# linhthi/BLISS-GNN

Measured on AMD Instinct MI355X. Metric: steps/sec (train step: sample_blocks + gather + SAGE fwd/bwd + Adam + exp3), reddit-like, higher is better.
Workload: dtype bf16

## Files before the change

bliss_gnn_amd/csrc/exp3.hip:

```cpp
#include "common.cuh"
#include "bliss_gnn.h"
#include "prof.h"
#include <cstdlib>

namespace {

#define E3_TPB 256
#ifndef NORM_NT
#define NORM_NT 1
#endif
#ifndef NORM_UNROLL
#define NORM_UNROLL 4
#endif

__device__ __forceinline__ void row_digits(bf16_t b, int64_t d[3], int* bad) {
  uint32_t e = (b >> 7) & 0xff, m = b & 0x7f;
  d[0] = d[1] = d[2] = 0;
  if (e == 255 || (b & 0x8000 && (b & 0x7fff))) { *bad |= BLISS_ERR_NONFINITE; return; }
  if (e == 0) e = 1; else m |= 0x80;
  int shift = (int)e - 134 + 64;
  if (shift > 80) { *bad |= BLISS_ERR_FIXED_RANGE; return; }
  if (shift < 0) { d[0] = (-shift >= 8) ? 0 : (int64_t)(m >> (-shift)); return; }
  const int idx = shift >> 5, off = shift & 31;
  const uint64_t v = (uint64_t)m << off;
  const int64_t lo = (int64_t)(v & 0xffffffffu), hi = (int64_t)(v >> 32);
  if (idx == 0) { d[0] = lo; d[1] = hi; }
  else if (idx == 1) { d[1] = lo; d[2] = hi; }
  else { d[2] = (int64_t)v; }
}

__device__ __forceinline__ int64_t wave_sum_i64(int64_t v) { return wave_total_i64(v); }

#define ROWSUM_SLOTS BLISS_ROWSUM_SLOTS
__device__ __forceinline__ void flush_digits(int64_t d[3], int64_t* limbs) {
  const int slot = (int)((blockIdx.x * (blockDim.x >> 6) + (threadIdx.x >> 6)) % ROWSUM_SLOTS);
#pragma unroll
  for (int i = 0; i < 3; ++i) {
    int64_t s = wave_sum_i64(d[i]);
    if (lane_id() == 0 && s != 0) atomicAdd((unsigned long long*)(limbs + 3 * slot + i), (unsigned long long)s);
  }
}
__device__ __forceinline__ void gather_limbs(const int64_t* limbs, int64_t out[3]) {
  out[0] = out[1] = out[2] = 0;
  for (int s = 0; s < ROWSUM_SLOTS; ++s) { out[0] += limbs[3 * s]; out[1] += limbs[3 * s + 1]; out[2] += limbs[3 * s + 2]; }
}

__device__ bf16_t limbs_to_bf16(const int64_t* replicas, int* bad) {
  int64_t limbs[3];
  gather_limbs(replicas, limbs);
  __int128 t = (__int128)limbs[0] + ((__int128)limbs[1] << 32) + ((__int128)limbs[2] << 64);
  if (t < 0) { *bad |= BLISS_ERR_FIXED_RANGE; return 0; }
  if (t == 0) return 0;
  unsigned __int128 u = (unsigned __int128)t;
  uint64_t hi = (uint64_t)(u >> 64), lo = (uint64_t)u;
  int msb = hi ? 127 - __clzll((long long)hi) : 63 - __clzll((long long)lo);
  unsigned __int128 q;
  if (msb > 7) {
    int sh = msb - 7;
    q = u >> sh;
    unsigned __int128 rem = u & ((((unsigned __int128)1) << sh) - 1), half = ((unsigned __int128)1) << (sh - 1);
    if (rem > half || (rem == half && (q & 1))) q += 1;
  } else q = u << (7 - msb);
  int e = msb - 64 + 127;
  if (q >= 256) { q >>= 1; e += 1; }
  if (e <= 0 || e >= 255) { *bad |= BLISS_ERR_FIXED_RANGE; return 0; }
  return (bf16_t)(((uint32_t)e << 7) | ((uint32_t)q & 0x7f));
}

__device__ __forceinline__ float nan_to_num_posinf0(float x) {
  if (x != x) return 0.f;
  if (x == __builtin_inff()) return 0.f;
  if (x == -__builtin_inff()) return -3.3895313892515355e38f;
  return x;
}

__device__ __forceinline__ void exp3_update_body(const int64_t* __restrict__ g_indptr, const bf16_t* __restrict__ edge_w,
                                                 bf16_t* w_row, int64_t* row_sum, const int* __restrict__ blk_indptr,
                                                 const int* __restrict__ blk_src, const int* __restrict__ blk_dst,
                                                 const int* __restrict__ blk_pos, const bf16_t* __restrict__ q_ij,
                                                 const bf16_t* __restrict__ node_prob, const bf16_t* __restrict__ embed_norm,
                                                 const bf16_t* __restrict__ alpha_in, const int* __restrict__ dst_nid,
                                                 const int* __restrict__ n_edges_dev, float delta_f,
                                                 bf16_t* __restrict__ rewards_out, bf16_t* __restrict__ factor_out,
                                                 int apply, int* err, int wg, int nwg, int bound) {
  int B = *n_edges_dev;
  int bad = 0;
  if (B > bound) { B = bound; bad |= BLISS_ERR_CAP_EDGES; }
  int64_t dg[3] = {0, 0, 0};
  for (int base = wg * E3_TPB + (threadIdx.x & ~63); base < B; base += nwg * E3_TPB) {
    const int e = base + lane_id();
    if (e < B) {
      const int i = blk_dst[e], j = blk_src[e], pos = blk_pos[e];
      const float alpha = bf2f(alpha_in ? alpha_in[e] : edge_w[pos]);
      const float k_i = rbf((float)(blk_indptr[i + 1] - blk_indptr[i]));
      float adk = rbf(rbf(alpha * alpha) / k_i);
      adk = nan_to_num_posinf0(adk);
      const float hn = bf2f(embed_norm[j]), q = bf2f(q_ij[e]);
      const float hq = rbf(rbf(hn * hn) / rbf(q * q));
      const float r = rbf(adk * hq);
      if (rewards_out) rewards_out[e] = f2bf(r);
      const int dn = dst_nid[i];
      const float n_i = rbf((float)(g_indptr[dn + 1] - g_indptr[dn]));
      const float r_hat = rbf(r / bf2f(node_prob[j]));
      float dr = rbf(r_hat * rbf(rbf(1.0f / n_i) * delta_f));
      if (dr > 1.0f) dr = 1.0f;
      const float ex = rbf((float)exp((double)dr));
      if (factor_out) factor_out[e] = f2bf(ex);
      if (!apply) continue;
      const bf16_t w_old = w_row[pos];
      const bf16_t w_new = f2bf(bf2f(w_old) * ex);
      if (w_new != w_old) {
        w_row[pos] = w_new;
        int64_t a[3], b[3];
        row_digits(w_new, a, &bad);
        row_digits(w_old, b, &bad);
        dg[0] += a[0] - b[0]; dg[1] += a[1] - b[1]; dg[2] += a[2] - b[2];
      }
    }
  }
  flush_digits(dg, row_sum);
  if (bad) atomicOr(err, bad);
}

__global__ void __launch_bounds__(E3_TPB) k_exp3_update(const int64_t* __restrict__ g_indptr, const bf16_t* __restrict__ edge_w,
                                                       bf16_t* w_row, int64_t* row_sum, const int* __restrict__ blk_indptr,
                                                       const int* __restrict__ blk_src, const int* __restrict__ blk_dst,
                                                       const int* __restrict__ blk_pos, const bf16_t* __restrict__ q_ij,
                                                       const bf16_t* __restrict__ node_prob, const bf16_t* __restrict__ embed_norm,
                                                       const bf16_t* __restrict__ alpha_in, const int* __restrict__ dst_nid,
                                                       const int* __restrict__ n_edges_dev, float delta_f,
                                                       bf16_t* __restrict__ rewards_out, bf16_t* __restrict__ factor_out,
                                                       int apply, int* err, int edges_bound) {
  exp3_update_body(g_indptr, edge_w, w_row, row_sum, blk_indptr, blk_src, blk_dst, blk_pos, q_ij, node_prob, embed_norm, alpha_in,
                   dst_nid, n_edges_dev, delta_f, rewards_out, factor_out, apply, err, blockIdx.x, gridDim.x, edges_bound);
}

struct Exp3Multi {
  bliss_exp3_block_t blk[BLISS_EXP3_MAX_BLOCKS];
  int grid_begin[BLISS_EXP3_MAX_BLOCKS + 1];
  int n;
};
__global__ void __launch_bounds__(E3_TPB) k_exp3_update_multi(const int64_t* __restrict__ g_indptr, const bf16_t* __restrict__ edge_w,
                                                             const Exp3Multi m, float delta_f, int* err) {
  int b = 0;
  while (b + 1 < m.n && (int)blockIdx.x >= m.grid_begin[b + 1]) ++b;
  const bliss_exp3_block_t& k = m.blk[b];
  exp3_update_body(g_indptr, edge_w, (bf16_t*)k.w_pos, k.row_sum, k.blk_indptr, k.blk_src, k.blk_dst, k.blk_pos, (const bf16_t*)k.q_ij,
                   (const bf16_t*)k.node_prob, (const bf16_t*)k.embed_norm, (const bf16_t*)k.alpha_or_null, k.dst_nid, k.n_edges_dev,
                   delta_f, (bf16_t*)k.rewards_out, nullptr, 1, err, (int)blockIdx.x - m.grid_begin[b], m.grid_begin[b + 1] - m.grid_begin[b],
                   k.edges_bound);
}

__global__ void __launch_bounds__(E3_TPB) k_exp3_apply(bf16_t* w_row, int64_t* row_sum, const int* __restrict__ pos,
                                                      const bf16_t* __restrict__ factor, const int* __restrict__ n_dev, int* err) {
  const int n = *n_dev;
  int bad = 0;
  int64_t dg[3] = {0, 0, 0};
  for (int e = blockIdx.x * E3_TPB + threadIdx.x; e < n; e += gridDim.x * E3_TPB) {
    const int p = pos[e];
    const bf16_t w_old = w_row[p];
    const bf16_t w_new = f2bf(bf2f(w_old) * bf2f(factor[e]));
    if (w_new != w_old) {
      w_row[p] = w_new;
      int64_t a[3], b[3];
      row_digits(w_new, a, &bad);
      row_digits(w_old, b, &bad);
      dg[0] += a[0] - b[0]; dg[1] += a[1] - b[1]; dg[2] += a[2] - b[2];
    }
  }
  flush_digits(dg, row_sum);
  if (bad) atomicOr(err, bad);
}

#define APPLY_MAX_WGS 256
struct ApplyLists {
  bf16_t* w_row[BLISS_EXP3_MAX_BLOCKS];
  int64_t* row_sum[BLISS_EXP3_MAX_BLOCKS];
  int pos_off[BLISS_EXP3_MAX_BLOCKS], fac_off[BLISS_EXP3_MAX_BLOCKS], cnt_off[BLISS_EXP3_MAX_BLOCKS], bound[BLISS_EXP3_MAX_BLOCKS];
  int n_blocks, n_ranks;
  long long rank_stride;
};

__global__ void __launch_bounds__(E3_TPB) k_exp3_apply_ranks(ApplyLists m, const int* __restrict__ gathered, int* bar, int* err) {
  int bad = 0;
  int64_t dg[BLISS_EXP3_MAX_BLOCKS][3];
#pragma unroll
  for (int b = 0; b < BLISS_EXP3_MAX_BLOCKS; ++b) dg[b][0] = dg[b][1] = dg[b][2] = 0;
  const int G = gridDim.x;
  for (int r = 0; r < m.n_ranks; ++r) {
    const int* base = gathered + (long long)r * m.rank_stride;
#pragma unroll
    for (int b = 0; b < BLISS_EXP3_MAX_BLOCKS; ++b) {
      if (b >= m.n_blocks) break;
      int n = base[m.cnt_off[b]];
      if (n > m.bound[b]) { n = m.bound[b]; bad |= BLISS_ERR_CAP_EDGES; }
      const int* pos = base + m.pos_off[b];
      const bf16_t* fac = reinterpret_cast<const bf16_t*>(base) + m.fac_off[b];
      for (int e = blockIdx.x * E3_TPB + threadIdx.x; e < n; e += G * E3_TPB) {
        const float f = bf2f(fac[e]);
        const uintptr_t a = (uintptr_t)(m.w_row[b] + pos[e]);
        unsigned* word = reinterpret_cast<unsigned*>(a & ~(uintptr_t)3);
        const int sh = (a & 2) ? 16 : 0;
        unsigned cur = __hip_atomic_load(word, __ATOMIC_RELAXED, __HIP_MEMORY_SCOPE_AGENT);
        for (;;) {
          const bf16_t w_old = (bf16_t)((cur >> sh) & 0xffffu);
          const bf16_t w_new = f2bf(bf2f(w_old) * f);
          if (w_new == w_old) break;
          const unsigned want = (cur & ~(0xffffu << sh)) | ((unsigned)w_new << sh);
          if (__hip_atomic_compare_exchange_strong(word, &cur, want, __ATOMIC_RELAXED, __ATOMIC_RELAXED, __HIP_MEMORY_SCOPE_AGENT)) {
            int64_t x[3], y[3];
            row_digits(w_new, x, &bad);
            row_digits(w_old, y, &bad);
            dg[b][0] += x[0] - y[0]; dg[b][1] += x[1] - y[1]; dg[b][2] += x[2] - y[2];
            break;
          }
        }
      }
    }
    if (r + 1 < m.n_ranks) {
      __syncthreads();
      if (threadIdx.x == 0) {
        __hip_atomic_fetch_add(bar, 1, __ATOMIC_RELEASE, __HIP_MEMORY_SCOPE_AGENT);
        long long spins = 0;
        while (__hip_atomic_load(bar, __ATOMIC_ACQUIRE, __HIP_MEMORY_SCOPE_AGENT) < (r + 1) * G) {
          __builtin_amdgcn_s_sleep(2);
          if (++spins > (1ll << 24)) { bad |= BLISS_ERR_FLAG_TIMEOUT; break; }
        }
      }
      __syncthreads();
    }
  }
#pragma unroll
  for (int b = 0; b < BLISS_EXP3_MAX_BLOCKS; ++b)
    if (b < m.n_blocks) flush_digits(dg[b], m.row_sum[b]);
  if (bad) atomicOr(err, bad);
  __syncthreads();
  if (threadIdx.x == 0 && __hip_atomic_fetch_add(bar + 1, 1, __ATOMIC_RELAXED, __HIP_MEMORY_SCOPE_AGENT) == G - 1) {
    __hip_atomic_store(bar, 0, __ATOMIC_RELAXED, __HIP_MEMORY_SCOPE_AGENT);
    __hip_atomic_store(bar + 1, 0, __ATOMIC_RELAXED, __HIP_MEMORY_SCOPE_AGENT);
  }
}

struct PackLists {
  const int* pos[BLISS_EXP3_MAX_BLOCKS];
  const int* n_dev[BLISS_EXP3_MAX_BLOCKS];
  int pos_off[BLISS_EXP3_MAX_BLOCKS], cnt_off[BLISS_EXP3_MAX_BLOCKS], bound[BLISS_EXP3_MAX_BLOCKS];
  int n_blocks;
};
__global__ void __launch_bounds__(E3_TPB) k_pack_lists(PackLists m, int* __restrict__ buf) {
  for (int b = 0; b < m.n_blocks; ++b) {
    const int n_true = *m.n_dev[b];
    const int n = n_true < m.bound[b] ? n_true : m.bound[b];
    if (blockIdx.x == 0 && threadIdx.x == 0) buf[m.cnt_off[b]] = n_true;
    const int* __restrict__ src = m.pos[b];
    int* __restrict__ dst = buf + m.pos_off[b];
    for (int e = blockIdx.x * E3_TPB + threadIdx.x; e < n; e += gridDim.x * E3_TPB) dst[e] = src[e];
  }
}

__global__ void __launch_bounds__(E3_TPB) k_row_sum(const bf16_t* __restrict__ w, int64_t n, int64_t* limbs, int* err) {
  int bad = 0;
  int64_t dg[3] = {0, 0, 0};
  for (int64_t i = (int64_t)blockIdx.x * E3_TPB + threadIdx.x; i < n; i += (int64_t)gridDim.x * E3_TPB) {
    int64_t a[3];
    row_digits(w[i], a, &bad);
    dg[0] += a[0]; dg[1] += a[1]; dg[2] += a[2];
  }
  flush_digits(dg, limbs);
  if (bad && err) atomicOr(err, bad);
}

__global__ void k_zero_i64(int64_t* p, int n) { if ((int)threadIdx.x < n) p[threadIdx.x] = 0; }

__device__ __forceinline__ float renorm_denom(bf16_t norm) { return rbf(fmaxf(bf2f(norm), 1e-12f)); }
__device__ __forceinline__ bf16_t renorm_bf16(bf16_t x, float denom) { return f2bf(bf2f(x) / denom); }

struct PairSlow { uint32_t word; int bad; int64_t d0, d1, d2; };
__device__ __attribute__((noinline)) PairSlow renorm_pair_slow(uint32_t word, float denom) {
  PairSlow r;
  r.bad = 0;
  const bf16_t lo = renorm_bf16((bf16_t)(word & 0xffffu), denom), hi = renorm_bf16((bf16_t)(word >> 16), denom);
  int64_t a[3], b[3];
  row_digits(lo, a, &r.bad);
  row_digits(hi, b, &r.bad);
  r.d0 = a[0] + b[0]; r.d1 = a[1] + b[1]; r.d2 = a[2] + b[2];
  r.word = (uint32_t)lo | ((uint32_t)hi << 16);
  return r;
}

__device__ __forceinline__ void normalize_row_body(bf16_t* w, int64_t n, int64_t* row_sum, int64_t* scratch, bf16_t* norm_out, int wg, int nwg,
                                                   const int64_t* norm_src = nullptr) {
  __shared__ int sh_norm, sh_last;
  if (threadIdx.x == 0) {
    int bad = 0;
    const bf16_t nb = limbs_to_bf16(norm_src ? norm_src : row_sum, &bad);
    sh_norm = (int)nb | (bad << 20);
    if (wg == 0) {
      scratch[0] = (int64_t)nb | ((int64_t)(nb == 0x3f80) << 16) | ((int64_t)bad << 20);
      if (norm_out) *norm_out = nb;
    }
  }
  __syncthreads();
  const bf16_t nb = (bf16_t)(sh_norm & 0xffff);
  if (nb == 0x3f80) return;
  const float denom = renorm_denom(nb);
  int bad = 0;
  int64_t dg[3] = {0, 0, 0};
  __shared__ int sh_tbl[128];
  if (threadIdx.x < 128) {
    const bf16_t x0 = (bf16_t)(0x3f80u | threadIdx.x);
    sh_tbl[threadIdx.x] = ((int)renorm_bf16(x0, denom) - (int)x0) & 0xffff;
  }
  const int de_lo = (int)(renorm_bf16((bf16_t)0x3f80u, denom) >> 7) - 127;
  const int de_hi = (int)(renorm_bf16((bf16_t)0x3fffu, denom) >> 7) - 127;
  const bool tbl_ok = de_lo > -126 && de_hi < 126 && de_lo <= de_hi;
  const uint32_t e_lo = (uint32_t)max(2, 2 - de_lo), e_hi = (uint32_t)min(253, 253 - de_hi);
  const int f_lo = max((int)e_lo, 70 - de_lo), f_hi = min((int)e_hi, 125 - de_hi);
  const bool pair_ok = tbl_ok && e_hi >= e_lo && f_hi >= f_lo;
  typedef unsigned short u16x2 __attribute__((ext_vector_type(2)));
  const unsigned short f_base = pair_ok ? (unsigned short)f_lo : (unsigned short)0xffffu, f_span = pair_ok ? (unsigned short)(f_hi - f_lo) : (unsigned short)0;
  const u16x2 FLO2 = {f_base, f_base}, SPAN2 = {f_span, f_span};
  __shared__ unsigned sh_bins[7][E3_TPB];
#pragma unroll
  for (int a = 0; a < 7; ++a) sh_bins[a][threadIdx.x] = 0;
  __syncthreads();
  auto one = [&](bf16_t x) {
    const bf16_t v = renorm_bf16(x, denom);
    int64_t a[3];
    row_digits(v, a, &bad);
    dg[0] += a[0]; dg[1] += a[1]; dg[2] += a[2];
    return v;
  };
  const int64_t head = min(n, (int64_t)(((16 - ((uintptr_t)w & 15)) & 15) >> 1));
  const int64_t nvec = (n - head) / 8;
  const int64_t gtid = (int64_t)wg * E3_TPB + threadIdx.x, gsz = (int64_t)nwg * E3_TPB;
  if (gtid < head) w[gtid] = one(w[gtid]);
  for (int64_t i = head + nvec * 8 + gtid; i < n; i += gsz) w[i] = one(w[i]);
  typedef unsigned int u32x4 __attribute__((ext_vector_type(4)));
  u32x4* wv = reinterpret_cast<u32x4*>(w + head);
#pragma unroll NORM_UNROLL
  for (int64_t i = gtid; i < nvec; i += gsz) {
#if NORM_NT
    u32x4 x = __builtin_nontemporal_load(wv + i);
#else
    u32x4 x = wv[i];
#endif
#pragma unroll
    for (int k = 0; k < 4; ++k) {
      const uint32_t word = x[k];
      const u16x2 W = __builtin_bit_cast(u16x2, word);
      const u16x2 D = (W >> 7) - FLO2;
      if (__builtin_bit_cast(uint32_t, __builtin_elementwise_max(D, SPAN2)) == __builtin_bit_cast(uint32_t, SPAN2)) {
        const uint32_t t = (uint32_t)sh_tbl[word & 0x7fu] | ((uint32_t)sh_tbl[(word >> 16) & 0x7fu] << 16);
        const u16x2 V = W + __builtin_bit_cast(u16x2, t);
        const uint32_t v2 = __builtin_bit_cast(uint32_t, V);
        const u16x2 S = (V >> 7) - (u16x2){70, 70};
        const u16x2 M = __builtin_bit_cast(u16x2, (v2 & 0x007f007fu) | 0x00800080u);
        const u16x2 T = M << (S & (u16x2){7, 7});
        const u16x2 A = S >> 3;
        __hip_atomic_fetch_add(&sh_bins[A.x][threadIdx.x], (unsigned)T.x, __ATOMIC_RELAXED, __HIP_MEMORY_SCOPE_WORKGROUP);
        __hip_atomic_fetch_add(&sh_bins[A.y][threadIdx.x], (unsigned)T.y, __ATOMIC_RELAXED, __HIP_MEMORY_SCOPE_WORKGROUP);
        x[k] = v2;
      } else {
        const PairSlow r = renorm_pair_slow(word, denom);
        x[k] = r.word; bad |= r.bad;
        dg[0] += r.d0; dg[1] += r.d1; dg[2] += r.d2;
      }
    }
#if NORM_NT == 1
    __builtin_nontemporal_store(x, wv + i);
#else
    wv[i] = x;
#endif
  }
  {
    uint64_t a = 0, b = 0;
#pragma unroll
    for (int k = 0; k < 4; ++k) a += (uint64_t)sh_bins[k][threadIdx.x] << (8 * k);
#pragma unroll
    for (int k = 4; k < 7; ++k) b += (uint64_t)sh_bins[k][threadIdx.x] << (8 * (k - 4));
    dg[0] += (int64_t)(a & 0xffffffffull); dg[1] += (int64_t)(a >> 32);
    dg[1] += (int64_t)(b & 0xffffffffull); dg[2] += (int64_t)(b >> 32);
  }
  flush_digits(dg, scratch + 2);
  if (bad) atomicOr((unsigned long long*)scratch, (unsigned long long)bad << 20);
  asm volatile("s_waitcnt vmcnt(0)" ::: "memory");
  __syncthreads();
  if (threadIdx.x == 0) sh_last = (atomicAdd((unsigned long long*)(scratch + 1), 1ull) == (unsigned long long)nwg - 1);
  __syncthreads();
  if (sh_last) {
    for (int k = threadIdx.x; k < 3 * ROWSUM_SLOTS; k += E3_TPB) {
      row_sum[k] = (int64_t)__hip_atomic_load((unsigned long long*)(scratch + 2 + k), __ATOMIC_RELAXED, __HIP_MEMORY_SCOPE_AGENT);
      __hip_atomic_store((unsigned long long*)(scratch + 2 + k), 0ull, __ATOMIC_RELAXED, __HIP_MEMORY_SCOPE_AGENT);
    }
    if (threadIdx.x == 0) __hip_atomic_store((unsigned long long*)(scratch + 1), 0ull, __ATOMIC_RELAXED, __HIP_MEMORY_SCOPE_AGENT);
  }
}

__global__ void __launch_bounds__(E3_TPB) k_normalize_row(bf16_t* w, int64_t n, int64_t* row_sum, int64_t* scratch, bf16_t* norm_out,
                                                          const int64_t* norm_src) {
  normalize_row_body(w, n, row_sum, scratch, norm_out, blockIdx.x, gridDim.x, norm_src);
}
__global__ void __launch_bounds__(E3_TPB) k_normalize_rows_global(const Exp3Multi m, int64_t n, int per_row, const int64_t* __restrict__ limbs,
                                                                  int64_t limb_stride) {
  const int r = blockIdx.x / per_row;
  const bliss_exp3_block_t& k = m.blk[r];
  normalize_row_body((bf16_t*)k.w_pos, n, k.row_sum, k.scratch, (bf16_t*)k.norm_out, (int)blockIdx.x - r * per_row, per_row, limbs + r * limb_stride);
}
__global__ void __launch_bounds__(E3_TPB) k_normalize_rows(const Exp3Multi m, int64_t n, int per_row) {
  const int r = blockIdx.x / per_row;
  const bliss_exp3_block_t& k = m.blk[r];
  normalize_row_body((bf16_t*)k.w_pos, n, k.row_sum, k.scratch, (bf16_t*)k.norm_out, (int)blockIdx.x - r * per_row, per_row);
}

__global__ void __launch_bounds__(E3_TPB) k_normalized_edata(const int64_t* __restrict__ indptr, int num_nodes, bf16_t* __restrict__ out) {
  const int lane = lane_id();
  for (int v = blockIdx.x * (E3_TPB / 64) + (threadIdx.x >> 6); v < num_nodes; v += gridDim.x * (E3_TPB / 64)) {
    const int64_t b = indptr[v], e = indptr[v + 1];
    const bf16_t val = f2bf(1.0f / rbf((float)(e - b)));
    for (int64_t p = b + lane; p < e; p += 64) out[p] = val;
  }
}

}

static int norm_wgs() {
  static const int v = [] { const char* e = getenv("BLISS_NORM_WGS"); int x = e ? atoi(e) : 0; return x > 0 ? x : 1024; }();
  return v;
}

extern "C" {

int bliss_exp3_update(const bliss_graph_t* g, const void* edge_w_pos, void* w_pos, int64_t* row_sum,
                      const int32_t* blk_indptr, const int32_t* blk_src, const int32_t* blk_dst,
                      const int32_t* blk_pos, const void* q_ij, const void* node_prob, const void* embed_norm,
                      const void* alpha_or_null, const int32_t* dst_nid, int32_t n_dst, const int32_t* n_edges_dev,
                      int32_t edges_bound, float delta_f, void* rewards_out, void* factor_out, int apply,
                      int32_t* err, void* stream) {
  if (!g || !w_pos || !row_sum || !blk_indptr || !blk_src || !blk_dst || !blk_pos || !q_ij || !node_prob ||
      !embed_norm || !dst_nid || !n_edges_dev || !err || (!edge_w_pos && !alpha_or_null))
    return BLISS_EINVAL;
  (void)n_dst;
  if (edges_bound <= 0) return 0;
  int grid = (edges_bound + E3_TPB - 1) / E3_TPB;
  if (grid > 2048) grid = 2048;
  hipStream_t st = (hipStream_t)stream;
  PROF_LAUNCH(BK_EXP3_UPDATE, st, k_exp3_update<<<grid, E3_TPB, 0, st>>>(g->indptr, (const bf16_t*)edge_w_pos, (bf16_t*)w_pos, row_sum, blk_indptr,
                                                          blk_src, blk_dst, blk_pos, (const bf16_t*)q_ij, (const bf16_t*)node_prob,
                                                          (const bf16_t*)embed_norm, (const bf16_t*)alpha_or_null, dst_nid,
                                                          n_edges_dev, delta_f, (bf16_t*)rewards_out, (bf16_t*)factor_out, apply, err, edges_bound));
  return (int)hipGetLastError();
}
// ... 160 lines not shown
```

bliss_gnn_amd/csrc/spmm.hip:

```cpp
#include "common.cuh"
#include "bliss_gnn.h"
#include "prof.h"

extern "C" int bliss_spmm_chunk_edges(int32_t nnz_bound);

namespace {

#define SP_TPB 256

struct f4 { float x, y, z, w; };

__device__ __forceinline__ int bcast_i(int v, int j) { return __builtin_amdgcn_readlane(v, j); }
__device__ __forceinline__ float bcast_f(float v, int j) { return __int_as_float(__builtin_amdgcn_readlane(__float_as_int(v), j)); }

__device__ __forceinline__ f4 load4(const bf16_t* p) {
  uint2 v = *reinterpret_cast<const uint2*>(p);
  f4 r;
  r.x = __uint_as_float(v.x << 16); r.y = __uint_as_float(v.x & 0xffff0000u);
  r.z = __uint_as_float(v.y << 16); r.w = __uint_as_float(v.y & 0xffff0000u);
  return r;
}

template <bool OUT_F32>
__device__ __forceinline__ void store4(void* out, int64_t off, f4 a) {
  if (OUT_F32) {
    *reinterpret_cast<float4*>((float*)out + off) = make_float4(a.x, a.y, a.z, a.w);
  } else {
    uint2 v;
    v.x = (uint32_t)f2bf(a.x) | ((uint32_t)f2bf(a.y) << 16);
    v.y = (uint32_t)f2bf(a.z) | ((uint32_t)f2bf(a.w) << 16);
    *reinterpret_cast<uint2*>((bf16_t*)out + off) = v;
  }
}


template <bool VEC4, bool OUT_F32>
__device__ __forceinline__ void store_row(void* out, int64_t off, f4 a, float scale) {
  a.x *= scale; a.y *= scale; a.z *= scale; a.w *= scale;
  if (VEC4) store4<OUT_F32>(out, off, a);
  else if (OUT_F32) ((float*)out)[off] = a.x;
  else ((bf16_t*)out)[off] = f2bf(a.x);
}

template <bool VEC4, bool OUT_F32, bool BWD>
__global__ void __launch_bounds__(SP_TPB) k_spmm(const int* __restrict__ row_ptr, const int* __restrict__ t_edge,
                                                const int* __restrict__ src, const int* __restrict__ dst,
                                                const int* __restrict__ blk_indptr, const bf16_t* __restrict__ w,
                                                const bf16_t* __restrict__ h, int64_t h_stride, int n_rows,
                                                const int* __restrict__ nnz_dev, int nnz_host, int dim,
                                                int mean, void* out, int64_t out_stride, float* __restrict__ part, int EC) {
  const int nnz = nnz_dev ? min(*nnz_dev, nnz_host) : nnz_host;
  const int lane = lane_id();
  const int chunk = blockIdx.x * (SP_TPB / 64) + (threadIdx.x >> 6);
  const int nchunks = nnz > 0 ? (nnz + EC - 1) / EC : 1;
  if (chunk >= nchunks) return;
  const int c0 = chunk * EC, c1 = min(nnz, c0 + EC), cnt = c1 - c0;
  int my_row = -1, my_n = 0;
  float my_c = 0.f;
  if (lane < cnt) {
    const int e = BWD ? t_edge[c0 + lane] : c0 + lane;
    my_row = BWD ? src[e] : dst[e];
    my_n = BWD ? dst[e] : src[e];
    float c = w ? bf2f(w[e]) : 1.0f;
    if (BWD && mean) { const int d = dst[e]; c = c / (float)max(blk_indptr[d + 1] - blk_indptr[d], 1); }
    my_c = c;
  }
  constexpr int W = VEC4 ? 4 : 1;
  const f4 zero = {0.f, 0.f, 0.f, 0.f};
  for (int col0 = 0; col0 < dim; col0 += 64 * W) {
    const int col = col0 + lane * W;
    const bool act = col < dim;
    auto flush = [&](int r, f4 acc) {
      const int rb = row_ptr[r], re = row_ptr[r + 1];
      const bool starts = rb >= c0, ends = re <= c1;
      if (!act) return;
      if (starts && ends) {
        const float scale = (!BWD && mean) ? 1.0f / (float)max(re - rb, 1) : 1.0f;
        store_row<VEC4, OUT_F32>(out, r * out_stride + col, acc, scale);
      } else {
        float* q = part + ((int64_t)chunk * 2 + (starts ? 1 : 0)) * dim + col;
        q[0] = acc.x;
        if (VEC4) { q[1] = acc.y; q[2] = acc.z; q[3] = acc.w; }
      }
    };
    if (cnt == 0) continue;
    int cur = bcast_i(my_row, 0);
    f4 acc = zero;
    for (int j = 0; j < cnt;) {
      const int r = bcast_i(my_row, j);
      if (r != cur) { flush(cur, acc); acc = zero; cur = r; }
      const int run = __popcll(__ballot(my_row == r && lane >= j));
      const int end = j + run;
      for (; j + 4 <= end; j += 4) {
        int n0 = bcast_i(my_n, j), n1 = bcast_i(my_n, j + 1), n2 = bcast_i(my_n, j + 2), n3 = bcast_i(my_n, j + 3);
        float k0 = bcast_f(my_c, j), k1 = bcast_f(my_c, j + 1), k2 = bcast_f(my_c, j + 2), k3 = bcast_f(my_c, j + 3);
        if (act) {
          if (VEC4) {
            f4 a0 = load4(h + n0 * h_stride + col), a1 = load4(h + n1 * h_stride + col);
            f4 a2 = load4(h + n2 * h_stride + col), a3 = load4(h + n3 * h_stride + col);
            acc.x += k0 * a0.x; acc.y += k0 * a0.y; acc.z += k0 * a0.z; acc.w += k0 * a0.w;
            acc.x += k1 * a1.x; acc.y += k1 * a1.y; acc.z += k1 * a1.z; acc.w += k1 * a1.w;
            acc.x += k2 * a2.x; acc.y += k2 * a2.y; acc.z += k2 * a2.z; acc.w += k2 * a2.w;
            acc.x += k3 * a3.x; acc.y += k3 * a3.y; acc.z += k3 * a3.z; acc.w += k3 * a3.w;
          } else {
            float a0 = bf2f(h[n0 * h_stride + col]), a1 = bf2f(h[n1 * h_stride + col]);
            float a2 = bf2f(h[n2 * h_stride + col]), a3 = bf2f(h[n3 * h_stride + col]);
            acc.x += k0 * a0; acc.x += k1 * a1; acc.x += k2 * a2; acc.x += k3 * a3;
          }
        }
      }
      for (; j < end; ++j) {
        int n0 = bcast_i(my_n, j);
        float k0 = bcast_f(my_c, j);
        if (act) {
          if (VEC4) {
            f4 a0 = load4(h + n0 * h_stride + col);
            acc.x += k0 * a0.x; acc.y += k0 * a0.y; acc.z += k0 * a0.z; acc.w += k0 * a0.w;
          } else acc.x += k0 * bf2f(h[n0 * h_stride + col]);
        }
      }
    }
    flush(cur, acc);
  }
}

template <bool OUT_F32, bool BWD, bool VEC4>
__global__ void __launch_bounds__(SP_TPB) k_spmm_fixup(const int* __restrict__ row_ptr, int n_rows, int dim, int mean,
                                                      const float* __restrict__ part, void* out, int64_t out_stride, int EC) {
  const int lane = lane_id();
  const int r = blockIdx.x * (SP_TPB / 64) + (threadIdx.x >> 6);
  if (r >= n_rows) return;
  const int rb = row_ptr[r], re = row_ptr[r + 1];
  constexpr int W = VEC4 ? 4 : 1;
  const f4 zero = {0.f, 0.f, 0.f, 0.f};
  if (re <= rb) {
    for (int col = lane * W; col < dim; col += 64 * W) store_row<VEC4, OUT_F32>(out, r * out_stride + col, zero, 1.0f);
    return;
  }
  const int c = rb / EC, c_end = (re - 1) / EC;
  if (c_end == c) return;
  const float scale = (!BWD && mean) ? 1.0f / (float)(re - rb) : 1.0f;
  for (int col = lane * W; col < dim; col += 64 * W) {
    f4 sum = zero;
    if (VEC4) {
      const float4 v = *reinterpret_cast<const float4*>(part + ((int64_t)c * 2 + 1) * dim + col);
      sum.x = v.x; sum.y = v.y; sum.z = v.z; sum.w = v.w;
#pragma unroll 4
      for (int cc = c + 1; cc <= c_end; ++cc) {
        const float4 u = *reinterpret_cast<const float4*>(part + ((int64_t)cc * 2) * dim + col);
        sum.x += u.x; sum.y += u.y; sum.z += u.z; sum.w += u.w;
      }
    } else {
      sum.x = part[((int64_t)c * 2 + 1) * dim + col];
      for (int cc = c + 1; cc <= c_end; ++cc) sum.x += part[((int64_t)cc * 2) * dim + col];
    }
    store_row<VEC4, OUT_F32>(out, r * out_stride + col, sum, scale);
  }
}

__global__ void __launch_bounds__(SP_TPB) k_embed_norm(const bf16_t* __restrict__ h, int n_rows, int dim, int64_t stride,
                                                      bf16_t* __restrict__ out, int vec4) {
  const int lane = lane_id();
  const int row = blockIdx.x * (SP_TPB / 64) + (threadIdx.x >> 6);
  if (row >= n_rows) return;
  const bf16_t* p = h + row * stride;
  float s = 0.f;
  if (vec4) {
    for (int c = lane * 4; c < dim; c += 256) {
      f4 a = load4(p + c);
      s += a.x * a.x; s += a.y * a.y; s += a.z * a.z; s += a.w * a.w;
    }
  } else {
    for (int c = lane; c < dim; c += 64) { float a = bf2f(p[c]); s += a * a; }
  }
  for (int d = 32; d >= 1; d >>= 1) s += __shfl_xor(s, d);
  if (lane == 0) out[row] = f2bf(sqrtf(s));
}

template <int W>
__global__ void __launch_bounds__(SP_TPB) k_gather_rows_norm(const bf16_t* __restrict__ feat, int64_t f_stride, const int* __restrict__ ids,
                                                            int n_rows, int dim, bf16_t* __restrict__ out, int64_t o_stride,
                                                            bf16_t* __restrict__ norm_out, int norm_vec4) {
  extern __shared__ __attribute__((aligned(16))) bf16_t rows_sh[];
  const int lane = lane_id(), wave = threadIdx.x >> 6;
  const int row = blockIdx.x * (SP_TPB / 64) + wave;
  if (row >= n_rows) return;
  const int dpad = (dim + 7) & ~7;
  bf16_t* sh = rows_sh + (size_t)wave * dpad;
  const bf16_t* p = feat + (int64_t)ids[row] * f_stride;
  bf16_t* q = out + (int64_t)row * o_stride;
  if (W == 4) {
    for (int c = lane * 4; c < dim; c += 256) { const uint2 v = *reinterpret_cast<const uint2*>(p + c); *reinterpret_cast<uint2*>(q + c) = v; *reinterpret_cast<uint2*>(sh + c) = v; }
  } else if (W == 2) {
    for (int c = lane * 2; c < dim; c += 128) { const uint32_t v = *reinterpret_cast<const uint32_t*>(p + c); *reinterpret_cast<uint32_t*>(q + c) = v; *reinterpret_cast<uint32_t*>(sh + c) = v; }
  } else {
    for (int c = lane; c < dim; c += 64) { const bf16_t v = p[c]; q[c] = v; sh[c] = v; }
  }
  if (!norm_out) return;
  __builtin_amdgcn_fence(__ATOMIC_RELEASE, "wavefront");
  __builtin_amdgcn_wave_barrier();
  float s = 0.f;
  if (norm_vec4) {
    for (int c = lane * 4; c < dim; c += 256) {
      const float a = bf2f(sh[c]), b = bf2f(sh[c + 1]), cc = bf2f(sh[c + 2]), d = bf2f(sh[c + 3]);
      s += a * a; s += b * b; s += cc * cc; s += d * d;
    }
  } else {
    for (int c = lane; c < dim; c += 64) { const float a = bf2f(sh[c]); s += a * a; }
  }
  for (int d = 32; d >= 1; d >>= 1) s += __shfl_xor(s, d);
  if (lane == 0) norm_out[row] = f2bf(sqrtf(s));
}

__device__ __forceinline__ uint32_t drop_hash(uint32_t seed, uint32_t ctr, uint32_t idx) {
  uint32_t x = idx * 0x9e3779b1u + seed;
  x ^= ctr * 0x85ebca77u + 0x165667b1u;
  x ^= x >> 16; x *= 0x7feb352du; x ^= x >> 15; x *= 0x846ca68bu; x ^= x >> 16;
  x += ctr; x ^= x >> 15; x *= 0x2c1b3c6du; x ^= x >> 12;
  return x;
}

template <bool VEC4>
__global__ void __launch_bounds__(SP_TPB) k_sage_epilogue(const bf16_t* __restrict__ a, int64_t a_stride, const bf16_t* __restrict__ b,
                                                         int64_t b_stride, int n_rows, int dim, uint32_t drop_thresh, float scale,
                                                         uint32_t seed, unsigned long long* ctr, bf16_t* __restrict__ out,
                                                         int64_t out_stride, bf16_t* __restrict__ norm_out) {
  const int lane = lane_id();
  const int row = blockIdx.x * (SP_TPB / 64) + (threadIdx.x >> 6);
  const uint32_t c = drop_thresh ? (uint32_t)__hip_atomic_load(ctr, __ATOMIC_RELAXED, __HIP_MEMORY_SCOPE_AGENT) : 0u;
  if (row < n_rows) {
    const bf16_t *pa = a + row * a_stride, *pb = b + row * b_stride;
    bf16_t* po = out + row * out_stride;
    float s = 0.f;
    constexpr int W = VEC4 ? 4 : 1;
    for (int col = lane * W; col < dim; col += 64 * W) {
      float v[W];
      if (VEC4) {
        const f4 x = load4(pa + col), y = load4(pb + col);
        v[0] = x.x + y.x; v[1 % W] = x.y + y.y; v[2 % W] = x.z + y.z; v[3 % W] = x.w + y.w;
      } else v[0] = bf2f(pa[col]) + bf2f(pb[col]);
#pragma unroll
      for (int i = 0; i < W; ++i) {
        float t = rbf(v[i]);
        t = t > 0.f ? t : 0.f;
        if (drop_thresh) {
          const bool keep = drop_hash(seed, c, (uint32_t)(row * dim + col + i)) >= drop_thresh;
          t = keep ? rbf(t * scale) : 0.f;
        }
        v[i] = t;
        s += t * t;
      }
      if (VEC4) {
        uint2 o;
        o.x = (uint32_t)f2bf(v[0]) | ((uint32_t)f2bf(v[1 % W]) << 16);
        o.y = (uint32_t)f2bf(v[2 % W]) | ((uint32_t)f2bf(v[3 % W]) << 16);
        *reinterpret_cast<uint2*>(po + col) = o;
      } else po[col] = f2bf(v[0]);
    }
    for (int d = 32; d >= 1; d >>= 1) s += __shfl_xor(s, d);
    if (lane == 0 && norm_out) norm_out[row] = f2bf(sqrtf(s));
  }
  if (drop_thresh) {
    __syncthreads();
    if (threadIdx.x == 0) {
      const unsigned G = gridDim.x < 64u ? gridDim.x : 64u, g = blockIdx.x % G;
      const unsigned long long members = (gridDim.x - g + G - 1) / G;
      if (atomicAdd(ctr + 2 + g, 1ull) == members - 1) {
        __hip_atomic_store(ctr + 2 + g, 0ull, __ATOMIC_RELAXED, __HIP_MEMORY_SCOPE_AGENT);
        if (atomicAdd(ctr + 1, 1ull) == (unsigned long long)G - 1) {
          __hip_atomic_store(ctr + 1, 0ull, __ATOMIC_RELAXED, __HIP_MEMORY_SCOPE_AGENT);
          atomicAdd(ctr, 1ull);
        }
      }
    }
  }
}

template <bool VEC4>
__global__ void __launch_bounds__(SP_TPB) k_sage_epilogue_bwd(const bf16_t* __restrict__ dout, int64_t d_stride, const bf16_t* __restrict__ out,
                                                             int64_t out_stride, int n_rows, int dim, float scale,
                                                             bf16_t* __restrict__ din, int64_t din_stride) {
  const int lane = lane_id();
  const int row = blockIdx.x * (SP_TPB / 64) + (threadIdx.x >> 6);
  if (row >= n_rows) return;
  constexpr int W = VEC4 ? 4 : 1;
  for (int col = lane * W; col < dim; col += 64 * W) {
    if (VEC4) {
      const f4 g = load4(dout + row * d_stride + col), o = load4(out + row * out_stride + col);
      f4 r;
      r.x = o.x > 0.f ? g.x * scale : 0.f; r.y = o.y > 0.f ? g.y * scale : 0.f;
      r.z = o.z > 0.f ? g.z * scale : 0.f; r.w = o.w > 0.f ? g.w * scale : 0.f;
      store4<false>(din, row * din_stride + col, r);
    } else {
      const float g = bf2f(dout[row * d_stride + col]);
      din[row * din_stride + col] = f2bf(bf2f(out[row * out_stride + col]) > 0.f ? g * scale : 0.f);
    }
  }
}

template <bool BWD>
int launch_spmm(const int* row_ptr, const int* t_edge, const int* src, const int* dst, const int* blk_indptr, const void* w,
                const void* h, int64_t h_stride, int n_rows, const int* nnz_dev, int nnz, int dim, int mean, void* out,
                int64_t out_stride, int out_fp32, float* part, hipStream_t st) {
  if (n_rows <= 0 || dim <= 0) return 0;
  const int EC = bliss_spmm_chunk_edges(nnz);
  if (nnz > EC && !part) return BLISS_EINVAL;
  const bool vec4 = (dim % 4 == 0) && (h_stride % 4 == 0) && (out_stride % 4 == 0) &&
                    (((uintptr_t)h) % 8 == 0) && (((uintptr_t)out) % (out_fp32 ? 16 : 8) == 0);
  const int nchunks = nnz > 0 ? (nnz + EC - 1) / EC : 1;
  dim3 grid((nchunks + SP_TPB / 64 - 1) / (SP_TPB / 64)), block(SP_TPB), gfix((n_rows + SP_TPB / 64 - 1) / (SP_TPB / 64));
#define GO(V, F) PROF_LAUNCH(BWD ? BK_SPMM_BWD : BK_SPMM_FWD, st, k_spmm<V, F, BWD><<<grid, block, 0, st>>>(row_ptr, t_edge, src, dst, blk_indptr, (const bf16_t*)w, (const bf16_t*)h, h_stride, n_rows, nnz_dev, nnz, dim, mean, out, out_stride, part, EC))
  if (vec4) { if (out_fp32) GO(true, true); else GO(true, false); }
  else      { if (out_fp32) GO(false, true); else GO(false, false); }
#undef GO
  {
    const bool fv = vec4 && (((uintptr_t)part) % 16 == 0);
#define FIX(F, V) PROF_LAUNCH(BK_SPMM_FIXUP, st, k_spmm_fixup<F, BWD, V><<<gfix, block, 0, st>>>(row_ptr, n_rows, dim, mean, part, out, out_stride, EC))
    if (out_fp32) { if (fv) FIX(true, true); else FIX(true, false); }
    else          { if (fv) FIX(false, true); else FIX(false, false); }
#undef FIX
  }
  return (int)hipGetLastError();
}

}

extern "C" {

int bliss_spmm_chunk_edges(int32_t nnz_bound) { return nnz_bound >= 200000 ? 64 : (nnz_bound >= 50000 ? 32 : 16); }

int bliss_spmm_fwd(const int32_t* indptr, const int32_t* src, const int32_t* dst, const void* w, const void* h,
                   int64_t h_stride, int32_t n_dst, const int32_t* nnz_dev, int32_t nnz, int32_t dim, int mean, void* out,
                   int64_t out_stride, int out_fp32, float* partials, void* stream) {
  if (!indptr || !h || !out || nnz < 0 || (nnz > 0 && (!src || !dst))) return BLISS_EINVAL;
  return launch_spmm<false>(indptr, nullptr, src, dst, nullptr, w, h, h_stride, n_dst, nnz_dev, nnz, dim, mean, out, out_stride, out_fp32,
                            partials, (hipStream_t)stream);
}

int bliss_spmm_bwd(const int32_t* t_indptr, const int32_t* t_edge, const int32_t* src, const int32_t* dst,
                   const int32_t* indptr, const void* w, const void* gout, int64_t gout_stride, int32_t n_src,
                   const int32_t* nnz_dev, int32_t nnz, int32_t dim, int mean, void* gh, int64_t gh_stride, int out_fp32,
                   float* partials, void* stream) {
  if (!t_indptr || !indptr || !gout || !gh || nnz < 0 || (nnz > 0 && (!t_edge || !src || !dst))) return BLISS_EINVAL;
  return launch_spmm<true>(t_indptr, t_edge, src, dst, indptr, w, gout, gout_stride, n_src, nnz_dev, nnz, dim, mean, gh, gh_stride,
                           out_fp32, partials, (hipStream_t)stream);
}

int bliss_sage_epilogue_fwd(const void* a, int64_t a_stride, const void* b, int64_t b_stride, int32_t n_rows, int32_t dim,
                            float p_drop, uint32_t seed, uint64_t* ctr, void* out, int64_t out_stride, void* norm_out, void* stream) {
  if (!a || !b || !out || n_rows < 0 || dim <= 0 || p_drop < 0.f || p_drop >= 1.f || (p_drop > 0.f && !ctr)) return BLISS_EINVAL;
  if (n_rows == 0) return 0;
  const bool v4 = dim % 4 == 0 && a_stride % 4 == 0 && b_stride % 4 == 0 && out_stride % 4 == 0 && ((uintptr_t)a) % 8 == 0 &&
                  ((uintptr_t)b) % 8 == 0 && ((uintptr_t)out) % 8 == 0;
  const uint32_t thresh = p_drop > 0.f ? (uint32_t)((double)p_drop * 4294967296.0) : 0u;
  const float scale = p_drop > 0.f ? 1.0f / (1.0f - p_drop) : 1.0f;
  hipStream_t st = (hipStream_t)stream;
  const int grid = (n_rows + SP_TPB / 64 - 1) / (SP_TPB / 64);
  if (v4) k_sage_epilogue<true><<<grid, SP_TPB, 0, st>>>((const bf16_t*)a, a_stride, (const bf16_t*)b, b_stride, n_rows, dim, thresh, scale, seed,
                                                        (unsigned long long*)ctr, (bf16_t*)out, out_stride, (bf16_t*)norm_out);
  else k_sage_epilogue<false><<<grid, SP_TPB, 0, st>>>((const bf16_t*)a, a_stride, (const bf16_t*)b, b_stride, n_rows, dim, thresh, scale, seed,
                                                      (unsigned long long*)ctr, (bf16_t*)out, out_stride, (bf16_t*)norm_out);
  return (int)hipGetLastError();
}

int bliss_sage_epilogue_bwd(const void* dout, int64_t dout_stride, const void* out, int64_t out_stride, int32_t n_rows, int32_t dim,
                            float p_drop, void* din, int64_t din_stride, void* stream) {
  if (!dout || !out || !din || n_rows < 0 || dim <= 0 || p_drop < 0.f || p_drop >= 1.f) return BLISS_EINVAL;
  if (n_rows == 0) return 0;
  const bool v4 = dim % 4 == 0 && dout_stride % 4 == 0 && out_stride % 4 == 0 && din_stride % 4 == 0 && ((uintptr_t)dout) % 8 == 0 &&
                  ((uintptr_t)out) % 8 == 0 && ((uintptr_t)din) % 8 == 0;
  const float scale = p_drop > 0.f ? 1.0f / (1.0f - p_drop) : 1.0f;
  hipStream_t st = (hipStream_t)stream;
  const int grid = (n_rows + SP_TPB / 64 - 1) / (SP_TPB / 64);
  if (v4) k_sage_epilogue_bwd<true><<<grid, SP_TPB, 0, st>>>((const bf16_t*)dout, dout_stride, (const bf16_t*)out, out_stride, n_rows, dim, scale,
                                                            (bf16_t*)din, din_stride);
  else k_sage_epilogue_bwd<false><<<grid, SP_TPB, 0, st>>>((const bf16_t*)dout, dout_stride, (const bf16_t*)out, out_stride, n_rows, dim, scale,
                                                          (bf16_t*)din, din_stride);
  return (int)hipGetLastError();
}

int bliss_gather_rows(const void* feat, int64_t feat_stride, const int32_t* ids, int32_t n_rows, int32_t dim, void* out,
                      int64_t out_stride, void* norm_out, void* stream) {
  if (!feat || !ids || !out || dim <= 0 || feat_stride < dim || out_stride < dim) return BLISS_EINVAL;
  if (n_rows <= 0) return 0;
  const size_t lds = (size_t)(SP_TPB / 64) * ((dim + 7) & ~7) * sizeof(bf16_t);
  if (lds > 48 * 1024) return BLISS_EINVAL;
  hipStream_t st = (hipStream_t)stream;
  const int grid = (n_rows + SP_TPB / 64 - 1) / (SP_TPB / 64);
  const uintptr_t al = (uintptr_t)feat | (uintptr_t)out;
  const int norm_vec4 = (dim % 4 == 0) && (out_stride % 4 == 0) && (((uintptr_t)out) % 8 == 0);
  if (dim % 4 == 0 && feat_stride % 4 == 0 && out_stride % 4 == 0 && al % 8 == 0)
    k_gather_rows_norm<4><<<grid, SP_TPB, lds, st>>>((const bf16_t*)feat, feat_stride, ids, n_rows, dim, (bf16_t*)out, out_stride, (bf16_t*)norm_out, norm_vec4);
  else if (dim % 2 == 0 && feat_stride % 2 == 0 && out_stride % 2 == 0 && al % 4 == 0)
    k_gather_rows_norm<2><<<grid, SP_TPB, lds, st>>>((const bf16_t*)feat, feat_stride, ids, n_rows, dim, (bf16_t*)out, out_stride, (bf16_t*)norm_out, norm_vec4);
  else
    k_gather_rows_norm<1><<<grid, SP_TPB, lds, st>>>((const bf16_t*)feat, feat_stride, ids, n_rows, dim, (bf16_t*)out, out_stride, (bf16_t*)norm_out, norm_vec4);
  return (int)hipGetLastError();
}

int bliss_embed_norm(const void* h, int32_t n_rows, int32_t dim, int64_t row_stride, void* out, void* stream) {
  if (!h || !out) return BLISS_EINVAL;
  if (n_rows <= 0) return 0;
  const int vec4 = (dim % 4 == 0) && (row_stride % 4 == 0) && (((uintptr_t)h) % 8 == 0);
  hipStream_t st = (hipStream_t)stream;
  PROF_LAUNCH(BK_EMBED_NORM, st, k_embed_norm<<<(n_rows + 3) / 4, SP_TPB, 0, st>>>((const bf16_t*)h, n_rows, dim, row_stride, (bf16_t*)out, vec4));
  return (int)hipGetLastError();
}

}
```

Before: 1462.

## Batch neighbor row loads in SpMM and wave-parallelize row-sum limb gather

Adds a new SpMM kernel that issues up to SP_DEPTH independent neighbor feature loads before accumulating, so that memory latency overlaps across edges. The old streaming kernel is kept for very large edge counts. Separately, the normalization header now gathers replica limbs with one lane per slot and a wave reduction instead of a serial loop on thread 0. The grouped loads use more registers, which may lower occupancy.

```diff
diff --git a/bliss_gnn_amd/csrc/exp3.hip b/bliss_gnn_amd/csrc/exp3.hip
--- a/bliss_gnn_amd/csrc/exp3.hip
+++ b/bliss_gnn_amd/csrc/exp3.hip
@@ -45,9 +45,7 @@
   for (int s = 0; s < ROWSUM_SLOTS; ++s) { out[0] += limbs[3 * s]; out[1] += limbs[3 * s + 1]; out[2] += limbs[3 * s + 2]; }
 }
 
-__device__ bf16_t limbs_to_bf16(const int64_t* replicas, int* bad) {
-  int64_t limbs[3];
-  gather_limbs(replicas, limbs);
+__device__ bf16_t limb_totals_to_bf16(const int64_t limbs[3], int* bad) {
   __int128 t = (__int128)limbs[0] + ((__int128)limbs[1] << 32) + ((__int128)limbs[2] << 64);
   if (t < 0) { *bad |= BLISS_ERR_FIXED_RANGE; return 0; }
   if (t == 0) return 0;
@@ -65,6 +63,18 @@
   if (q >= 256) { q >>= 1; e += 1; }
   if (e <= 0 || e >= 255) { *bad |= BLISS_ERR_FIXED_RANGE; return 0; }
   return (bf16_t)(((uint32_t)e << 7) | ((uint32_t)q & 0x7f));
+}
+__device__ bf16_t limbs_to_bf16(const int64_t* replicas, int* bad) {
+  int64_t limbs[3];
+  gather_limbs(replicas, limbs);
+  return limb_totals_to_bf16(limbs, bad);
+}
+__device__ __forceinline__ void gather_limbs_wave(const int64_t* limbs, int64_t out[3]) {
+  static_assert(ROWSUM_SLOTS <= BLISS_WAVE, "one lane per replica");
+  const int s = lane_id();
+  int64_t l0 = 0, l1 = 0, l2 = 0;
+  if (s < ROWSUM_SLOTS) { l0 = limbs[3 * s]; l1 = limbs[3 * s + 1]; l2 = limbs[3 * s + 2]; }
+  out[0] = wave_sum_i64(l0); out[1] = wave_sum_i64(l1); out[2] = wave_sum_i64(l2);
 }
 
 __device__ __forceinline__ float nan_to_num_posinf0(float x) {
@@ -291,13 +301,17 @@
 __device__ __forceinline__ void normalize_row_body(bf16_t* w, int64_t n, int64_t* row_sum, int64_t* scratch, bf16_t* norm_out, int wg, int nwg,
                                                    const int64_t* norm_src = nullptr) {
   __shared__ int sh_norm, sh_last;
-  if (threadIdx.x == 0) {
-    int bad = 0;
-    const bf16_t nb = limbs_to_bf16(norm_src ? norm_src : row_sum, &bad);
-    sh_norm = (int)nb | (bad << 20);
-    if (wg == 0) {
-      scratch[0] = (int64_t)nb | ((int64_t)(nb == 0x3f80) << 16) | ((int64_t)bad << 20);
-      if (norm_out) *norm_out = nb;
+  if (threadIdx.x < BLISS_WAVE) {
+    int64_t tot[3];
+    gather_limbs_wave(norm_src ? norm_src : row_sum, tot);
+    if (threadIdx.x == 0) {
+      int bad = 0;
+      const bf16_t nb = limb_totals_to_bf16(tot, &bad);
+      sh_norm = (int)nb | (bad << 20);
+      if (wg == 0) {
+        scratch[0] = (int64_t)nb | ((int64_t)(nb == 0x3f80) << 16) | ((int64_t)bad << 20);
+        if (norm_out) *norm_out = nb;
+      }
     }
   }
   __syncthreads();
diff --git a/bliss_gnn_amd/csrc/spmm.hip b/bliss_gnn_amd/csrc/spmm.hip
--- a/bliss_gnn_amd/csrc/spmm.hip
+++ b/bliss_gnn_amd/csrc/spmm.hip
@@ -1,6 +1,7 @@
 #include "common.cuh"
 #include "bliss_gnn.h"
 #include "prof.h"
+#include <type_traits>
 
 extern "C" int bliss_spmm_chunk_edges(int32_t nnz_bound);
 
@@ -42,8 +43,105 @@
   else ((bf16_t*)out)[off] = f2bf(a.x);
 }
 
+#ifndef SP_DEPTH
+#define SP_DEPTH 16
+#endif
+
+__device__ __forceinline__ f4 unpack4(uint2 v) {
+  f4 r;
+  r.x = __uint_as_float(v.x << 16); r.y = __uint_as_float(v.x & 0xffff0000u);
+  r.z = __uint_as_float(v.y << 16); r.w = __uint_as_float(v.y & 0xffff0000u);
+  return r;
+}
+
 template <bool VEC4, bool OUT_F32, bool BWD>
 __global__ void __launch_bounds__(SP_TPB) k_spmm(const int* __restrict__ row_ptr, const int* __restrict__ t_edge,
+                                                const int* __restrict__ src, const int* __restrict__ dst,
+                                                const int* __restrict__ blk_indptr, const bf16_t* __restrict__ w,
+                                                const bf16_t* __restrict__ h, int64_t h_stride, int n_rows,
+                                                const int* __restrict__ nnz_dev, int nnz_host, int dim,
+                                                int mean, void* out, int64_t out_stride, float* __restrict__ part, int EC) {
+  const int nnz = nnz_dev ? min(*nnz_dev, nnz_host) : nnz_host;
+  const int lane = lane_id();
+  const int chunk = blockIdx.x * (SP_TPB / 64) + __builtin_amdgcn_readfirstlane(threadIdx.x >> 6);
+  const int nchunks = nnz > 0 ? (nnz + EC - 1) / EC : 1;
+  if (chunk >= nchunks) return;
+  const int c0 = chunk * EC, c1 = min(nnz, c0 + EC), cnt = c1 - c0;
+  int my_row = -1, my_n = 0, my_rb = 0, my_re = 0;
+  float my_c = 0.f;
+  if (lane < cnt) {
+    const int e = BWD ? t_edge[c0 + lane] : c0 + lane;
+    const int s = src[e], d = dst[e];
+    my_row = BWD ? s : d;
+    my_n = BWD ? d : s;
+    int ip0 = 0, ip1 = 1;
+    if (BWD && mean) { ip0 = blk_indptr[d]; ip1 = blk_indptr[d + 1]; }
+    my_rb = row_ptr[my_row]; my_re = row_ptr[my_row + 1];
+    float c = w ? bf2f(w[e]) : 1.0f;
+    if (BWD && mean) c = c / (float)max(ip1 - ip0, 1);
+    my_c = c;
+  }
+  if (cnt == 0) return;
+  constexpr int W = VEC4 ? 4 : 1;
+  constexpr int D = SP_DEPTH;
+  const f4 zero = {0.f, 0.f, 0.f, 0.f};
+  for (int col0 = 0; col0 < dim; col0 += 64 * W) {
+    const int col = col0 + lane * W;
+    const bool act = col < dim;
+    auto flush = [&](int jl, int r, f4 acc) {
+      const int rb = bcast_i(my_rb, jl), re = bcast_i(my_re, jl);
+      const bool starts = rb >= c0, ends = re <= c1;
+      if (!act) return;
+      if (starts && ends) {
+        const float scale = (!BWD && mean) ? 1.0f / (float)max(re - rb, 1) : 1.0f;
+        store_row<VEC4, OUT_F32>(out, r * out_stride + col, acc, scale);
+      } else {
+        float* q = part + ((int64_t)chunk * 2 + (starts ? 1 : 0)) * dim + col;
+        q[0] = acc.x;
+        if (VEC4) { q[1] = acc.y; q[2] = acc.z; q[3] = acc.w; }
+      }
+    };
+    int cur = bcast_i(my_row, 0);
+    f4 acc = zero;
+    auto group = [&](int g, auto full_tag) {
+      constexpr bool FULL = decltype(full_tag)::value;
+      uint2 v[D];
+      int nb[D];
+#pragma unroll
+      for (int i = 0; i < D; ++i) { v[i] = make_uint2(0u, 0u); nb[i] = bcast_i(my_n, g + i); }
+      if (act) {
+#pragma unroll
+        for (int i = 0; i < D; ++i) {
+          if (FULL || g + i < cnt) {
+            const bf16_t* p = h + nb[i] * h_stride + col;
+            if (VEC4) v[i] = *reinterpret_cast<const uint2*>(p);
+            else v[i].x = (uint32_t)*p;
+          }
+        }
+      }
+#pragma unroll
+      for (int i = 0; i < D; ++i) {
+        if (FULL || g + i < cnt) {
+          const int r = bcast_i(my_row, g + i);
+          if (r != cur) { flush(g + i - 1, cur, acc); acc = zero; cur = r; }
+          const float k = bcast_f(my_c, g + i);
+          if (VEC4) {
+            const f4 a = unpack4(v[i]);
+            acc.x += k * a.x; acc.y += k * a.y; acc.z += k * a.z; acc.w += k * a.w;
+          } else acc.x += k * bf2f((bf16_t)v[i].x);
+        }
+      }
+    };
+    int g = 0;
+    for (; g + D <= cnt; g += D) group(g, std::true_type{});
+    if (g < cnt) group(g, std::false_type{});
+    flush(cnt - 1, cur, acc);
+  }
+}
+
+#define SP_GROUPED_MAX_EDGES (1 << 20)
+template <bool VEC4, bool OUT_F32, bool BWD>
+__global__ void __launch_bounds__(SP_TPB) k_spmm_stream(const int* __restrict__ row_ptr, const int* __restrict__ t_edge,
                                                 const int* __restrict__ src, const int* __restrict__ dst,
                                                 const int* __restrict__ blk_indptr, const bf16_t* __restrict__ w,
                                                 const bf16_t* __restrict__ h, int64_t h_stride, int n_rows,
@@ -309,7 +407,7 @@
                     (((uintptr_t)h) % 8 == 0) && (((uintptr_t)out) % (out_fp32 ? 16 : 8) == 0);
   const int nchunks = nnz > 0 ? (nnz + EC - 1) / EC : 1;
   dim3 grid((nchunks + SP_TPB / 64 - 1) / (SP_TPB / 64)), block(SP_TPB), gfix((n_rows + SP_TPB / 64 - 1) / (SP_TPB / 64));
-#define GO(V, F) PROF_LAUNCH(BWD ? BK_SPMM_BWD : BK_SPMM_FWD, st, k_spmm<V, F, BWD><<<grid, block, 0, st>>>(row_ptr, t_edge, src, dst, blk_indptr, (const bf16_t*)w, (const bf16_t*)h, h_stride, n_rows, nnz_dev, nnz, dim, mean, out, out_stride, part, EC))
+#define GO(V, F) PROF_LAUNCH(BWD ? BK_SPMM_BWD : BK_SPMM_FWD, st, (nnz >= SP_GROUPED_MAX_EDGES ? k_spmm_stream<V, F, BWD> : k_spmm<V, F, BWD>)<<<grid, block, 0, st>>>(row_ptr, t_edge, src, dst, blk_indptr, (const bf16_t*)w, (const bf16_t*)h, h_stride, n_rows, nnz_dev, nnz, dim, mean, out, out_stride, part, EC))
   if (vec4) { if (out_fp32) GO(true, true); else GO(true, false); }
   else      { if (out_fp32) GO(false, true); else GO(false, false); }
 #undef GO
```

New measurement: 1475 (median of 6 runs). No clear change (+0.9%).
